# aiforvision/OCTA-autosegmentation

Measured on AMD Instinct MI355X. Metric: synthetic OCTA samples/sec (graph + 304x304 image + 1216x1216 label triples), higher is better.
Workload: dtype f64

## Files before the change

__graft_entry__.py:

```python
import os
import subprocess
import sys

ROOT = os.path.dirname(os.path.abspath(__file__))
if ROOT not in sys.path:
    sys.path.insert(0, ROOT)


def build() -> None:
    from octa_autosegmentation_amd import build as b
    lib = b.build()
    assert os.path.exists(lib)
    from oracle import octa_oracle
    octa_oracle.build()
    nat = os.path.join(ROOT, "tests", "native")
    subprocess.check_call(["g++", "-O2", "-std=c++17", "-ffp-contract=off", "-fPIC", "-shared", "-o",
                           os.path.join(nat, "libcorehost.so"), os.path.join(nat, "raster_core_host.cpp")])
    subprocess.check_call(["g++", "-O2", "-std=c++17", "-mfma", "-ffp-contract=off", "-fPIC", "-shared", "-o",
                           os.path.join(nat, "libsimcorehost.so"), os.path.join(nat, "sim_core_host.cpp")])
    subprocess.check_call(["g++", "-O2", "-std=c++17", "-mfma", "-ffp-contract=off", "-fPIC", "-shared", "-DOCTA_SIM_LARGE=1", "-o",
                           os.path.join(nat, "libsimcorehost_large.so"), os.path.join(nat, "sim_core_host.cpp")])
    import octa_autosegmentation_amd
    from octa_autosegmentation_amd import _native
    assert _native.lib().octa_abi_version() == 2


def smoke() -> None:
    import numpy as np
    import torch
    from octa_autosegmentation_amd.vessel_graph_generation import tree2img
    from oracle import octa_oracle
    assert torch.cuda.is_available(), "smoke() needs a GPU"
    torch.cuda.set_device(0)
    rng = np.random.default_rng(0)
    n = 500
    e = np.zeros((n, 7))
    e[:, 0:3] = rng.uniform(0, 1, (n, 3))
    e[:, 3:6] = e[:, 0:3] + rng.normal(0, 0.03, (n, 3))
    e[:, 6] = rng.uniform(0.001, 0.01, n)
    d = torch.from_numpy(e).cuda()
    img = tree2img.rasterize_edges_device(d, np.array([0, n]), [304, 304])
    lab = tree2img.binarize_label_device(img)
    torch.cuda.synchronize()
    ref = octa_oracle.rasterize(e, [304, 304])
    assert (img[0].cpu().numpy() == ref).all(), "HIP rasteriser differs from the oracle"
    assert (lab[0].cpu().numpy() == octa_oracle.fs_dither(ref)).all(), "HIP dither differs from the oracle"
    import yaml
    from octa_autosegmentation_amd import graph_io
    from octa_autosegmentation_amd.vessel_graph_generation import greenhouse
    from oracle import sim_oracle
    g = np.load(os.path.join(ROOT, "tests", "golden", "sim_golden.npz"))
    cfg = yaml.safe_load(str(g["config_yaml"]))
    cfg["Greenhouse"]["modes"][0]["I"] = 12
    cfg["Greenhouse"]["modes"][1]["I"] = 6
    res = greenhouse.simulate_batch(cfg, [3, 4])
    for k, seed in enumerate((3, 4)):
        e, _ = sim_oracle.simulate(cfg, seed)
        assert graph_io.edges_to_csv_text(res.sample_edges(k)) == sim_oracle.edges_to_csv_text(e), "HIP simulator differs from the oracle"
    import torch.nn.functional as F
    from octa_autosegmentation_amd.models import mfma_conv
    gen = torch.Generator(device="cuda").manual_seed(0)
    x = torch.randn(1, 24, 40, 32, device="cuda", generator=gen).to(torch.bfloat16)
    w = (torch.randn(64, 32, 3, 3, device="cuda", generator=gen) / 17.0).to(torch.bfloat16).float()
    xr, wr = x.float().permute(0, 3, 1, 2).requires_grad_(True), w.clone().requires_grad_(True)
    yr = F.conv2d(xr, wr, padding=1)
    dy = torch.randn(yr.shape, device="cuda", generator=gen).to(torch.bfloat16)
    yr.backward(dy.float())
    xm, wm = x.clone().requires_grad_(True), w.clone().requires_grad_(True)
    ym = mfma_conv.conv3x3(xm, wm, 1)
    ym.backward(dy.permute(0, 2, 3, 1).contiguous())
    tol = lambda a, b: (a.float() - b).abs().max().item() <= 2.0 ** -8 * b.abs().max().item() + 1e-6
    assert tol(ym.detach(), yr.detach().permute(0, 2, 3, 1)), "MFMA convolution differs from torch fp32"
    assert tol(xm.grad, xr.grad.permute(0, 2, 3, 1)), "MFMA data gradient differs from torch fp32"
    assert (wm.grad - wr.grad).abs().max().item() <= 1e-3 * wr.grad.abs().max().item(), "MFMA weight gradient differs from torch fp32"
    print("smoke ok: simulator CSV + raster + dither bit-exact vs oracle, MFMA conv fwd/dgrad/wgrad vs torch fp32, on", torch.cuda.get_device_name(0))


if __name__ == "__main__":
    build()
    if len(sys.argv) > 1 and sys.argv[1] == "smoke":
        smoke()
```

octa_autosegmentation_amd/csrc/sim_core.h:

```cpp
#pragma once
#include <cmath>
#include <cstdint>
#include <cstring>
#include <algorithm>
#include "gpow.h"
#include "glibc_trig.h"

#ifndef OCTA_SIM_LARGE
#define OCTA_SIM_LARGE 0
#endif
#if OCTA_SIM_LARGE
#define OCTA_SIMK octa_simk_large
#else
#define OCTA_SIMK octa_simk
#endif
namespace OCTA_SIMK {

#if OCTA_SIM_LARGE
typedef unsigned int idx_t;
typedef unsigned long long kdw_t;
constexpr int IDX_BITS = 18;
constexpr int GROUP_BITS = 17;
constexpr int NCAP = 1 << 17;
constexpr int OCAP = 1 << 18;
// ... 814 lines not shown
#pragma unroll
        for (int d = 1; d < 64; d <<= 1) {
            int u = __shfl_up(inc, d, 64);
            if (tl >= d) inc += u;
        }
        const int totS = __shfl(inc, 63, 64);
        const int preS = inc - nS;
        const int cut = base + totS;
        {
            int g = (p0 - base) - preS;
            const int lim = p1 < cut ? p1 : cut;
            for (int i = p0; i < lim; i++)
                if (!kd_less_w(a, a.kv[i], pk)) box[g++] = (idx_t)i;
        }
        __builtin_amdgcn_wave_barrier();
        {
            int r = totS - preS - nS;
            const int lo = p0 > cut ? p0 : cut;
            for (int i = p1 - 1; i >= lo; i--)
                if (kd_less_w(a, a.kv[i], pk)) kd_swap(a, i, (int)box[r++]);
        }
        __builtin_amdgcn_wave_barrier();
        if (cut <= nth) first = cut; else last = cut;
    }
    kd_nth_element_team<64, 4>(a, first, nth, last, true, mb, depth);
}
#endif

OCTA_HD inline unsigned f32_bits(float v) { unsigned u; memcpy(&u, &v, 4); return u; }
OCTA_HD inline unsigned f32_sortable(float v) {
    unsigned u;
    memcpy(&u, &v, 4);
    return (u >> 31) ? ~u : (u | 0x80000000u);
}
OCTA_HD inline float f32_unsortable(unsigned e) {
    unsigned u = (e >> 31) ? (e & 0x7fffffffu) : ~e;
    float v;
    memcpy(&v, &u, 4);
    return v;
}
OCTA_HD inline float f32_round_up(double x) {
#if defined(__HIP_DEVICE_COMPILE__)
    return __double2float_ru(x);
#else
    float f = (float)x;
    return (double)f < x ? nextafterf(f, INFINITY) : f;
#endif
}
OCTA_HD inline float f32_round_down(double x) {
#if defined(__HIP_DEVICE_COMPILE__)
    return __double2float_rd(x);
#else
    float f = (float)x;
    return (double)f > x ? nextafterf(f, -INFINITY) : f;
#endif
}
OCTA_HD inline double f32_ulp(float v) {
    const float a = fabsf(v);
    return (double)nextafterf(a, INFINITY) - (double)a;
}
OCTA_HD inline void atomic_max_u32(unsigned *p, unsigned v) {
#if defined(__HIP_DEVICE_COMPILE__)
    atomicMax(p, v);
#else
    if (v > *p) *p = v;
#endif
}
OCTA_HD inline void atomic_min_u32(unsigned *p, unsigned v) {
#if defined(__HIP_DEVICE_COMPILE__)
    atomicMin(p, v);
#else
    if (v < *p) *p = v;
#endif
}

constexpr int KD_TAB_OFF = OCAP * (int)sizeof(kdw_t);
constexpr int KD_BOX_BYTES = KD_RANGES * 24;
static_assert(KD_RANGES >= OCAP / 17 + 1, "ranges per level");
static_assert(KD_MAILBOX_OFF % 16 == 0 && KD_MAILBOX_OFF >= KD_TAB_OFF + KD_RANGES * KD_TAB_BYTES_PER_RANGE, "kd tables overlap the mailbox");
static_assert(KD_MAILBOX_OFF + (KD_BOX_BYTES > KD_MAILBOX_BYTES ? KD_BOX_BYTES : KD_MAILBOX_BYTES) <= SIM_USER_BYTES, "kd table layout (box table and mailbox share their area)");
OCTA_HD inline void kd_build(const Blk &b, const double *pts, int n, idx_t *out_idx, idx_t *out_rank,
                              float *xy, double zlo, double zhi, long *kdprof = nullptr, const unsigned char *need = nullptr,
                              const bool flag_in_sign = false) {
#if defined(__HIP_DEVICE_COMPILE__) && !defined(OCTA_SIM_PROF_ASSIGN) && !defined(OCTA_SIM_PROF_SAMPLE) && !defined(OCTA_SIM_PROF_SET) && !defined(OCTA_SIM_PROF_MAIL) && !defined(OCTA_SIM_PROF_SEQ) && !defined(OCTA_SIM_PROF_SEQ2)
#define KDP(slot) do { if (kdprof && b.tid == 0) { long _t = (long)wall_clock64(); kdprof[slot] += _t - _kt; _kt = _t; } } while (0)
    long _kt = (long)wall_clock64();
#else
#define KDP(slot) do { } while (0)
#endif
    kdw_t *kv = reinterpret_cast<kdw_t *>(b.user_of<1>());
    idx_t *tab = reinterpret_cast<idx_t *>(b.user_of<1>() + KD_TAB_OFF);
    idx_t *rs = tab, *re = tab + KD_RANGES;
    idx_t *rs2 = tab + 2 * KD_RANGES, *re2 = tab + 3 * KD_RANGES;
    signed char *rd = reinterpret_cast<signed char *>(tab + 4 * KD_RANGES);
    unsigned *bbf = reinterpret_cast<unsigned *>(b.user_of<1>() + KD_MAILBOX_OFF);
#if defined(__HIP_DEVICE_COMPILE__) && !OCTA_SIM_LARGE
    if ((size_t)n * (sizeof(kdw_t) + 8) + 8 <= (size_t)KD_TAB_OFF)
        xy = reinterpret_cast<float *>(b.user_of<1>() + (((size_t)n * sizeof(kdw_t) + 7) & ~(size_t)7));
#endif
    for (int i = b.tid; i < n; i += b.nth) {
        kv[i] = (kdw_t)i;
        const float fx = (float)pts[3 * i];
        xy[2 * i] = (flag_in_sign && need[i]) ? -fx : fx; xy[2 * i + 1] = (float)pts[3 * i + 1];
    }
    if (b.tid == 0) { rs[0] = 0; re[0] = (idx_t)n; }
    const float z_up = f32_round_up(zhi), z_dn = f32_round_down(zlo);
    b.sync();
    int nr = (n > 16) ? 1 : 0;
    while (nr > 0) {
        for (int q = b.tid; q < nr; q += b.nth) {
            for (int k = 0; k < 2; k++) { bbf[6 * q + k] = 0u; bbf[6 * q + 3 + k] = ~0u; }
            bbf[6 * q + 2] = f32_sortable(z_up); bbf[6 * q + 5] = f32_sortable(z_dn);
            rd[q] = 0;
        }
        b.sync();
        {
            const int chunk = ((n + b.nth - 1) / b.nth) | 1;
            const int i0 = b.tid * chunk, i1 = (i0 + chunk < n) ? i0 + chunk : n;
            int q = 0;
            if (i0 < i1) {
                int lo_ = 0, hi_ = nr - 1;
                while (lo_ < hi_) { int mid = (lo_ + hi_ + 1) >> 1; if (rs[mid] <= i0) lo_ = mid; else hi_ = mid - 1; }
                q = lo_;
            }
            bool have = false, hit = false;
            float mx[2] = {0, 0}, mn[2] = {0, 0};
            auto flush = [&](int qq) {
                for (int k = 0; k < 2; k++) {
                    atomic_max_u32(&bbf[6 * qq + k], f32_sortable(nextafterf(mx[k], INFINITY)));
                    atomic_min_u32(&bbf[6 * qq + 3 + k], f32_sortable(nextafterf(mn[k], -INFINITY)));
                }
            };
            constexpr int KB = 8;
            int qw = q, cs = 0, ce = 0, ns = 0x7fffffff;
            if (i0 < i1) { cs = rs[qw]; ce = re[qw]; ns = qw + 1 < nr ? (int)rs[qw + 1] : 0x7fffffff; }
            for (int ib = i0; ib < i1; ib += KB) {
                int eq[KB], eid[KB];
                kdw_t ew[KB];
#pragma unroll
                for (int k = 0; k < KB; k++) ew[k] = kv[ib + k < i1 ? ib + k : i1 - 1];
#pragma unroll
                for (int k = 0; k < KB; k++) {
                    const int i = ib + k;
                    eq[k] = -1; eid[k] = 0;
                    if (i < i1) {
                        while (i >= ns) { qw++; cs = ns; ce = re[qw]; ns = qw + 1 < nr ? (int)rs[qw + 1] : 0x7fffffff; }
                        if (i >= cs && i < ce) { eq[k] = qw; eid[k] = (int)(ew[k] & KD_IDX_MASK); }
                    }
                }
                float ex[KB], ey[KB];
                unsigned char nd[KB];
#pragma unroll
                for (int k = 0; k < KB; k++) {
                    const float sx = xy[2 * eid[k]];
                    ex[k] = flag_in_sign ? fabsf(sx) : sx; ey[k] = xy[2 * eid[k] + 1];
                    nd[k] = flag_in_sign ? (unsigned char)(f32_bits(sx) >> 31) : (need ? need[eid[k]] : (unsigned char)1);
                }
#pragma unroll
                for (int k = 0; k < KB; k++) {
                    if (eq[k] < 0) continue;
                    if (eq[k] != q) {
                        if (have) { flush(q); have = false; }
                        if (hit) { rd[q] = 1; hit = false; }
                        q = eq[k];
                    }
                    if (nd[k]) hit = true;
                    if (!have) { mx[0] = mn[0] = ex[k]; mx[1] = mn[1] = ey[k]; }
// ... 110 lines not shown
                }
            }
        }
        b.sync();
        KDP(2);
#if defined(__HIP_DEVICE_COMPILE__)
        {
            idx_t *mb = reinterpret_cast<idx_t *>(b.user_of<1>() + KD_MAILBOX_OFF);
            const int wv = b.tid >> 6, nw = (b.nth + 63) >> 6;
            for (int q = wv; q < nr; q += nw) {
                int d = rd[q];
                int s = rs[q], e = re[q];
                if (d < 0 || e - s < KD_TEAM_MIN) continue;
                const KdPair kp = {kv, pts, d};
                if (e - s > KD_MASK_MAX) kd_nth_element_wave_long(kp, s, s + (e - s) / 2, e, mb);
                else if (e - s > 4000) kd_nth_element_team<64, 4>(kp, s, s + (e - s) / 2, e, true, mb);
                else kd_nth_element_team<64, 1>(kp, s, s + (e - s) / 2, e, true, mb);
            }
        }
        KDP(3);
        {
            idx_t *mb = reinterpret_cast<idx_t *>(b.user_of<1>() + KD_MAILBOX_OFF);
            const int team = b.tid >> 4, nteam = b.nth >> 4;
            for (int q0 = 0; q0 < nr; q0 += nteam) {
                int q = q0 + team;
                bool live = q < nr;
                int s = 0, e = 0, d = 0;
                if (live) {
                    s = rs[q]; e = re[q]; d = rd[q];
                    live = d >= 0 && e - s < KD_TEAM_MIN;
                }
                const KdPair kp = {kv, pts, d < 0 ? 0 : d};
                kd_nth_element_team<16, 1>(kp, s, s + (e - s) / 2, e, live, mb);
            }
        }
#else
        for (int q = b.tid; q < nr; q += b.nth) {
            int d = rd[q];
            if (d < 0) continue;
            int s = rs[q], e = re[q];
            const KdPair kp = {kv, pts, d};
            kd_nth_element(kp, s, s + (e - s) / 2, e);
        }
#endif
        b.sync();
        KDP(4);
        {
            int base = 0;
            for (int q0 = 0; q0 < nr; q0 += b.nth) {
                const int q = q0 + b.tid;
                int s = 0, e = 0, m = 0, c = 0;
                if (q < nr && rd[q] >= 0) {
                    s = rs[q]; e = re[q]; m = s + (e - s) / 2;
                    c = (m - s > 16 ? 1 : 0) + (e - m > 16 ? 1 : 0);
                }
                int ex;
                const int tot = blk_scan(b, c, &ex);
                int pos = base + ex;
                if (m - s > 16) { if (pos < KD_RANGES) { rs2[pos] = (idx_t)s; re2[pos] = (idx_t)m; } pos++; }
                if (e - m > 16) { if (pos < KD_RANGES) { rs2[pos] = (idx_t)m; re2[pos] = (idx_t)e; } }
                base += tot;
            }
            nr = base < KD_RANGES ? base : KD_RANGES;
        }
        { idx_t *t = rs; rs = rs2; rs2 = t; t = re; re = re2; re2 = t; }
        KDP(5);
    }
    for (int i = b.tid; i < n; i += b.nth) { const idx_t id = (idx_t)(kv[i] & KD_IDX_MASK); out_idx[i] = id; out_rank[id] = (idx_t)i; }
    b.sync();
    KDP(6);
#undef KDP
}


constexpr int GRID_N = NCAP > OCAP ? NCAP : OCAP;
struct Grid {
    int nx, ny;
    double x0, y0, inv, cell;
    const int *cell_end;
    const idx_t *items;
    const double *spts;
    const float *sptf;
    const double *src;
};
OCTA_HD inline int grid_clampi(int v, int hi) { return v < 0 ? 0 : (v > hi ? hi : v); }
OCTA_HD inline int grid_cx(const Grid &G, double x) { return grid_clampi((int)floor((x - G.x0) * G.inv), G.nx - 1); }
OCTA_HD inline int grid_cy(const Grid &G, double y) { return grid_clampi((int)floor((y - G.y0) * G.inv), G.ny - 1); }

OCTA_HD inline Grid grid_build_once(const Blk &b, const SimArrays &A, const double *pts, const int *ids, int n, double radius, int div, bool as_float,
                                    const unsigned char *mask) {
    Grid G;
    const double span = 1.2;
    double cell = fmax(radius / div, span / GRID_MAX);
    int nc = (int)ceil(span / cell);
    if (nc < 1) nc = 1;
    if (nc > GRID_MAX) nc = GRID_MAX;
    G.nx = G.ny = nc; G.x0 = G.y0 = -0.1; G.inv = 1.0 / cell; G.cell = cell;
    const int ncell = nc * nc;
    int *hist = reinterpret_cast<int *>(b.user_of<2>());
    idx_t *items = reinterpret_cast<idx_t *>(b.user_of<2>() + (size_t)(GRID_MAX * GRID_MAX + 1) * 4);
    static_assert((size_t)(GRID_MAX * GRID_MAX + 1) * 4 + (size_t)GRID_N * sizeof(idx_t) <= (size_t)SIM_USER_BYTES, "grid table layout");
    G.cell_end = hist; G.items = items; G.spts = A.grid_pts; G.sptf = reinterpret_cast<const float *>(A.grid_pts); G.src = pts;
    if (n > GRID_N) n = GRID_N;
    b.sync();
    for (int c = b.tid; c <= ncell; c += b.nth) hist[c] = 0;
    b.sync();
    constexpr int GB = 4;
    for (int i0 = b.tid; i0 < n; i0 += GB * b.nth) {
        double px[GB], py[GB];
        bool live[GB];
#pragma unroll
        for (int k = 0; k < GB; k++) {
            const int i = i0 + k * b.nth;
            const int ic = i < n ? i : n - 1;
            const double *p = pts + 3 * (ids ? ids[ic] : ic);
            px[k] = p[0]; py[k] = p[1];
            live[k] = i < n && (!mask || mask[ic]);
        }
#pragma unroll
        for (int k = 0; k < GB; k++)
            if (live[k]) atomic_add_int(&hist[grid_cy(G, py[k]) * nc + grid_cx(G, px[k])], 1);
    }
    b.sync();
    {
        const int total = ncell + 1;
        const int chunk = ((total + b.nth - 1) / b.nth) | 1;
        const int c0 = b.tid * chunk, c1 = (c0 + chunk < total) ? c0 + chunk : total;
        int local = 0;
        for (int c = c0; c < c1; c++) local += hist[c];
        int ex;
        blk_scan(b, local, &ex);
        int run = ex;
        for (int c = c0; c < c1; c++) { int v = hist[c]; hist[c] = run; run += v; }
    }
    b.sync();
    for (int i0 = b.tid; i0 < n; i0 += GB * b.nth) {
        V3 p[GB];
        int id[GB];
        bool live[GB];
#pragma unroll
        for (int k = 0; k < GB; k++) {
            const int i = i0 + k * b.nth;
            const int ic = i < n ? i : n - 1;
            id[k] = ids ? ids[ic] : ic;
            p[k] = ld3(pts + 3 * id[k]);
            live[k] = i < n && (!mask || mask[ic]);
        }
#pragma unroll
        for (int k = 0; k < GB; k++)
            if (live[k]) {
                int pos = atomic_add_int(&hist[grid_cy(G, p[k].y) * nc + grid_cx(G, p[k].x)], 1);
                items[pos] = (idx_t)id[k];
                if (as_float) { float *f = reinterpret_cast<float *>(A.grid_pts) + 3 * pos; f[0] = (float)p[k].x; f[1] = (float)p[k].y; f[2] = (float)p[k].z; }
                else st3(A.grid_pts + 3 * pos, p[k]);
            }
    }
    b.sync();
    return G;
}
OCTA_HD inline Grid grid_build(const Blk &b, const SimArrays &A, const double *pts, const int *ids, int n, double radius, int div = 1,
                               bool as_float = false, const unsigned char *mask = nullptr) {
#if OCTA_SIM_DUP & 2
    grid_build_once(b, A, pts, ids, n, radius, div, as_float, mask);
#endif
    return grid_build_once(b, A, pts, ids, n, radius, div, as_float, mask);
}
constexpr int GRID_VB = 4;
constexpr double GRID_F_TAU = 1e-6;
struct Pt3f { float x, y, z; };
OCTA_HD inline float sqdist_f(Pt3f a, float cx, float cy, float cz) { const float dx = a.x - cx, dy = a.y - cy, dz = a.z - cz; return fmaf(dz, dz, fmaf(dy, dy, dx * dx)); }
template <bool FLT> struct GridPt;
template <> struct GridPt<false> { typedef V3 T; static OCTA_HD inline V3 load(const Grid &G, int k) { return ld3(G.spts + 3 * k); } static OCTA_HD inline V3 zero() { return v3(0, 0, 0); } };
template <> struct GridPt<true> {
    typedef Pt3f T;
    static OCTA_HD inline Pt3f load(const Grid &G, int k) { const float *f = G.sptf + 3 * k; Pt3f r = {f[0], f[1], f[2]}; return r; }
    static OCTA_HD inline Pt3f zero() { Pt3f r = {0.f, 0.f, 0.f}; return r; }
};
template <bool FLT, class F>
OCTA_HD inline void grid_visit_impl(const Grid &G, double px, double py, double radius, F &&body) {
    const int cy0 = grid_cy(G, py - radius), cy1 = grid_cy(G, py + radius);
    const int cx0 = grid_cx(G, px - radius), cx1 = grid_cx(G, px + radius);
    for (int cyb = cy0; cyb <= cy1; cyb += 3) {
        int k0[3], k1[3];
#pragma unroll
        for (int r = 0; r < 3; r++) {
            const int row = cyb + r;
            k0[r] = k1[r] = 0;
            if (row <= cy1) {
                const int c0 = row * G.nx + cx0;
                k0[r] = c0 ? G.cell_end[c0 - 1] : 0;
                k1[r] = G.cell_end[row * G.nx + cx1];
            }
        }
        typename GridPt<FLT>::T pt[3][GRID_VB];
        int it[3][GRID_VB];
#pragma unroll
        for (int r = 0; r < 3; r++)
#pragma unroll
            for (int u = 0; u < GRID_VB; u++) {
                const int k = k0[r] + u < k1[r] ? k0[r] + u : k0[r];
                pt[r][u] = k0[r] < k1[r] ? GridPt<FLT>::load(G, k) : GridPt<FLT>::zero();
                it[r][u] = k0[r] < k1[r] ? (int)G.items[k] : 0;
            }
#pragma unroll
        for (int r = 0; r < 3; r++) {
#pragma unroll
            for (int u = 0; u < GRID_VB; u++)
                if (k0[r] + u < k1[r]) body(it[r][u], pt[r][u]);
            for (int kb = k0[r] + GRID_VB; kb < k1[r]; kb += GRID_VB) {
                typename GridPt<FLT>::T q[GRID_VB];
                int iq[GRID_VB];
#pragma unroll
                for (int u = 0; u < GRID_VB; u++) {
                    const int k = kb + u < k1[r] ? kb + u : kb;
                    q[u] = GridPt<FLT>::load(G, k);
                    iq[u] = (int)G.items[k];
                }
#pragma unroll
                for (int u = 0; u < GRID_VB; u++)
                    if (kb + u < k1[r]) body(iq[u], q[u]);
            }
        }
    }
}
template <class F>
OCTA_HD inline void grid_visit(const Grid &G, double px, double py, double radius, F &&body) { grid_visit_impl<false>(G, px, py, radius, body); }
template <class F>
OCTA_HD inline void grid_visit_f(const Grid &G, double px, double py, double radius, F &&body) { grid_visit_impl<true>(G, px, py, radius, body); }

struct DirtyList {
    int *v;
    int n, cap;
    bool overflow;
};
OCTA_HD inline void dirty_insert(DirtyList &D, int g) {
    int i = 0;
    while (i < D.n && D.v[i] < g) i++;
    if (i < D.n && D.v[i] == g) return;
    if (OCTA_UNLIKELY(D.n >= D.cap)) { D.overflow = true; return; }
    for (int k = D.n; k > i; k--) D.v[k] = D.v[k - 1];
    D.v[i] = g;
    D.n++;
}

struct SeqLds {
    double *rad;
    idx_t *par;
    const double *log_tab;
    const uint64_t *exp_tab;
    int *deferred;
    int *changed;
    double *fl_val;
    int *fl_done;
    int *slot_of;
};
#ifndef OCTA_MURRAY_EPT
#define OCTA_MURRAY_EPT 4
#endif
constexpr int MURRAY_EPT = OCTA_MURRAY_EPT;
constexpr int MURRAY_FLUSH_WAVE = MURRAY_EPT * 64;
constexpr int MURRAY_FLUSH_LDS = 3 * MURRAY_FLUSH_WAVE;
constexpr int PAR_BITS = (int)sizeof(idx_t) * 8 - 2;
constexpr unsigned PAR_MASK = (1u << PAR_BITS) - 1u, PAR_DEF = 1u << PAR_BITS, PAR_TAG = 2u << PAR_BITS;
static_assert((unsigned)NCAP <= PAR_MASK, "node ids fit the parent field of a node word");
OCTA_HD inline bool changed_get(const SeqLds &L, int g) { return ((unsigned)L.changed[g >> 5] >> (g & 31)) & 1u; }
OCTA_HD inline void changed_set(const SeqLds &L, int g) { L.changed[g >> 5] |= (int)(1u << (g & 31)); }
OCTA_HD inline bool deferred_get(const SeqLds &L, int id) { return ((unsigned)L.deferred[id >> 5] >> (id & 31)) & 1u; }
struct WalkRec { int nch, c0, c1, cg; double k; };
OCTA_HD inline WalkRec walk_load(const SimArrays &A, int f, int id, bool want_cg) {
    WalkRec r;
    const int j = id < 0 ? 0 : id;
    r.nch = A.nnch_of(f)[j]; r.c0 = A.nch0_of(f)[j]; r.c1 = A.nch1_of(f)[j];
    r.cg = want_cg ? A.child_group[j] : 0;
    r.k = A.nkap_of(f)[j];
    return r;
}
OCTA_HD inline int walk_parent(const SeqLds &L, int id) {
    if (id < 0) return -1;
    const unsigned p = (unsigned)L.par[id] & PAR_MASK;
    return p == PAR_MASK ? -1 : (int)p;
}

#if defined(__HIP_DEVICE_COMPILE__)
__device__ inline double readlane_f64(double v, int j ) {
    int lo = __builtin_amdgcn_readlane(__double2loint(v), j), hi = __builtin_amdgcn_readlane(__double2hiint(v), j);
    return __hiloint2double(hi, lo);
}
__device__ inline bool murray_pending_above(const SimArrays &A, int start, int cur_g, int pass_tag, const SeqLds &L) {
    const int lane = (int)(threadIdx.x & 63);
    int cur = start;
    while (true) {
        int nn = 0, mine = -1;
        bool ended = false;
        for (; nn < 64; nn++) {
            const unsigned w = (unsigned)L.par[cur], p = w & PAR_MASK;
            if (p == PAR_MASK || (w & PAR_DEF)) { ended = true; break; }
            if (lane == nn) mine = cur;
            cur = (int)p;
        }
        const int cg = lane < nn ? A.child_group[mine] : 0;
        if (__ballot(lane < nn && (cg >> (GROUP_BITS + 1)) == pass_tag && (cg & ((1 << GROUP_BITS) - 1)) > cur_g)) return true;
        if (ended) return false;
    }
}
#ifdef OCTA_WALK_POW_LDS
#define OCTA_WALK_POW(x, y) octa_gpow::gpow_t((x), (y), L.log_tab, L.exp_tab)
#else
#define OCTA_WALK_POW(x, y) octa_gpow::gpow_u((x), (y))
#endif
__device__ inline long murray_to_root(const SimArrays &A, int f, int id, int cur_g, int pass_tag, DirtyList *D, const SeqLds &L, int &n_def
#ifdef OCTA_SIM_PROF_SEQ2
// ... 1397 lines not shown
#endif
        }
    }
    b.sync();
}

OCTA_HD inline void murray_flush_pending(const Blk &b, const SimArrays &A) {
#if defined(__HIP_DEVICE_COMPILE__)
    b.sync();
    double *fl_val = reinterpret_cast<double *>(b.user_of<8>());
    int *fl_done = reinterpret_cast<int *>(fl_val + MURRAY_FLUSH_LDS);
    for (int f = 0; f < 2; f++) {
        const int n = OCTA_UNI(A.sc->fl_pending[f]);
        if (n <= 0) continue;
        for (int i = b.tid; i < MURRAY_FLUSH_LDS / 32; i += b.nth) fl_done[i] = 0;
        b.sync();
        const int wv = b.tid >> 6;
        if (wv < 3 && wv * 64 < n) {
            const int rounds = murray_flush_rounds_wave(A.nrad_of(f), octa_gpow::LOG_TAB, octa_gpow::EXP_TAB, fl_val, fl_done, A.fl_rec + (size_t)f * MURRAY_FLUSH_LDS, n,
                                                        wv, 3, true);
            if (b.tid == 0) { A.sc->fl_pending[f] = 0; A.sc->flush_rounds += rounds; }
        }
        b.sync();
    }
#else
    (void)b; (void)A;
#endif
}

constexpr int COMPACT_TILE = 3072;
OCTA_HD inline int compact_points(const Blk &b, double *pts, int n, const unsigned char *removed, double *stage) {
    (void)stage;
    if (b.nth == 1) {
        int w = 0;
        for (int i = 0; i < n; i++)
            if (!removed[i]) { if (w != i) { pts[3 * w] = pts[3 * i]; pts[3 * w + 1] = pts[3 * i + 1]; pts[3 * w + 2] = pts[3 * i + 2]; } w++; }
        return w;
    }
    double *tile = reinterpret_cast<double *>(b.user_of<16>());
    static_assert((size_t)COMPACT_TILE * 24 <= (size_t)SIM_USER_BYTES, "compaction tile");
#if defined(__HIP_DEVICE_COMPILE__)
    const int lane = b.tid & 63, wv = b.tid >> 6, nw = (b.nth + 63) >> 6;
    int base = 0;
    for (int t0 = 0; t0 < n; t0 += COMPACT_TILE) {
        const int tn = n - t0 < COMPACT_TILE ? n - t0 : COMPACT_TILE;
        const int seg = ((tn + nw * 64 - 1) / (nw * 64)) * 64;
        const int s0 = t0 + (wv * seg < tn ? wv * seg : tn), s1 = s0 + seg < t0 + tn ? s0 + seg : t0 + tn;
        int c = 0;
        for (int i0 = s0; i0 < s1; i0 += 64) c += (int)__popcll(__ballot(i0 + lane < s1 && !removed[i0 + lane]));
        int ex;
        const int kept = blk_scan(b, lane == 0 ? c : 0, &ex);
        if (base != t0 || kept != tn) {
            int at = __builtin_amdgcn_readfirstlane(ex);
            for (int i0 = s0; i0 < s1; i0 += 64) {
                const bool keep = i0 + lane < s1 && !removed[i0 + lane];
                const unsigned long long m = __ballot(keep);
                if (keep) {
                    const int w = at + (int)__popcll(m & ((1ull << lane) - 1ull));
                    const V3 v = ld3(pts + 3 * (size_t)(i0 + lane));
                    tile[3 * w] = v.x; tile[3 * w + 1] = v.y; tile[3 * w + 2] = v.z;
                }
                at += (int)__popcll(m);
            }
            b.sync();
            for (int j = b.tid; j < kept * 3; j += b.nth) pts[(size_t)3 * base + j] = tile[j];
            b.sync();
        }
        base += kept;
    }
    return base;
#else
    (void)tile;
    return n;
#endif
}

#if defined(__HIP_DEVICE_COMPILE__)
#define OCTA_SUBPROF(sc, slot, t0) do { if (b.tid == 0) { long _t1 = (long)wall_clock64(); (sc)->prof[slot] += _t1 - (t0); (t0) = _t1; } } while (0)
#define OCTA_SUBPROF_T0() ((long)wall_clock64())
#else
#define OCTA_SUBPROF(sc, slot, t0) do { (void)(t0); } while (0)
#define OCTA_SUBPROF_T0() 0L
#endif

OCTA_HD inline void phase_satisfy_art(const Blk &b, const SimArrays &A, const SimConst &C, const IterParams &P) {
    const double zext = C.sz;
    SampleScalars *sc = A.sc;
    const int nb = sc->new_begin[0], ne = sc->new_end[0];
    const int n_new = ne - nb, n_oxy = sc->n_oxy;
    if (n_new <= 0 || n_oxy <= 0) return;
    const double ek = P.eps_k, ek2 = ek * ek;
    long t0 = OCTA_SUBPROF_T0();
    for (int i = b.tid; i < n_oxy; i += b.nth) A.removed[i] = 0;
    int *ctl = b.coll() + 100;
    if (b.tid == 0) { ctl[0] = 0; ctl[1] = 0; }
    b.sync();
    {
        int *new_ids = A.tmp_int;
        for (int j = b.tid; j < n_new; j += b.nth) new_ids[j] = nb + j;
        b.sync();
        Grid G = grid_build(b, A, A.npos[0], new_ids, n_new, ek);
        for (int o = b.tid; o < n_oxy; o += b.nth) {
            const V3 p = ld3(A.oxy + 3 * o);
            grid_visit(G, p.x, p.y, ek, [&](int j, const V3 &q) {
                if (sqdist(p, q) <= ek2) {
                    int slot = atomic_add_int(&ctl[0], 1);
                    if (slot < PCAP) A.pairs[slot] = ((unsigned)(j - nb) << IDX_BITS) | (unsigned)o;
                    A.removed[o] = 1;
                }
            });
        }
        b.sync();
    }
    OCTA_SUBPROF(sc, 12, t0);
    int n_pairs = ctl[0];
    if (n_pairs > PCAP) { if (b.tid == 0) atomic_or_int(&sc->err, ERR_PAIR_CAP); n_pairs = PCAP; }
    if (n_new > (1 << (32 - IDX_BITS))) { if (b.tid == 0) atomic_or_int(&sc->err, ERR_PAIR_CAP); }
    b.sync();
    if (n_pairs == 0) return;
    {
        const int n_ven = sc->n_nodes[1];
        int *rem = A.tmp_int;
        int n_rem = 0;
        {
            const int chunk = (n_oxy + b.nth - 1) / b.nth;
            const int i0 = b.tid * chunk < n_oxy ? b.tid * chunk : n_oxy, i1 = (i0 + chunk < n_oxy) ? i0 + chunk : n_oxy;
            int local = 0;
            for (int o = i0; o < i1; o++) local += A.removed[o] ? 1 : 0;
            int ex;
            n_rem = blk_scan(b, local, &ex);
            int run = ex;
            for (int o = i0; o < i1; o++) if (A.removed[o]) rem[run++] = o;
        }
        b.sync();
        for (int k = b.tid; k < n_rem; k += b.nth) {
            const int o = rem[k];
            A.ven_near[o] = 0;
            A.hashes[o] = py_hash_tuple3(ld3(A.oxy + 3 * o));
        }
        Grid G = grid_build(b, A, A.oxy, rem, n_rem, ek);
        constexpr int VB = 4;
        for (int j0 = b.tid; j0 < n_ven; j0 += VB * b.nth) {
            V3 qv[VB];
#pragma unroll
            for (int u = 0; u < VB; u++) { const int j = j0 + u * b.nth; qv[u] = ld3(A.npos[1] + 3 * (j < n_ven ? j : n_ven - 1)); }
#pragma unroll
            for (int u = 0; u < VB; u++) {
                if (j0 + u * b.nth >= n_ven) break;
                const V3 q = qv[u];
                grid_visit(G, q.x, q.y, ek, [&](int o, const V3 &p) {
                    if (sqrt(sqdist(q, p)) <= ek) A.ven_near[o] = 1;
                });
            }
        }
        b.sync();
    }
    OCTA_SUBPROF(sc, 12, t0);
    bool set_in_lds = false, ranked = false;
#ifdef OCTA_SIM_DEBUG_SAT
    int dbg_n_ins = -1, dbg_mask = -1, dbg_base = -1;
    const int dbg_n_co2_in = sc->n_co2;
#endif
    for (int pass = 0; pass < 2; pass++) {
        ranked = pass > 0;
        if (ranked) {
            kd_build(b, A.oxy, n_oxy, A.kd_idx, A.kd_rank, reinterpret_cast<float *>(A.tmp_dbl), 0.0, zext, sc->kdprof, A.removed, true);
#if OCTA_SIM_DUP & 1
            kd_build(b, A.oxy, n_oxy, A.kd_idx, A.kd_rank, reinterpret_cast<float *>(A.tmp_dbl), 0.0, zext, nullptr, A.removed, true);
#endif
            for (int i = b.tid; i < n_pairs; i += b.nth) {
                unsigned pr = A.pairs[i];
                A.pairs[i] = (pr & ~IDX_MASK) | (unsigned)A.kd_rank[pr & IDX_MASK];
            }
            b.sync();
            OCTA_SUBPROF(sc, 11, t0);
        }
        unsigned *keys = reinterpret_cast<unsigned *>(b.user_of<32>());
        int n_pow2 = 1;
        while (n_pow2 < n_pairs) n_pow2 <<= 1;
        for (int i = b.tid; i < n_pow2; i += b.nth) keys[i] = i < n_pairs ? A.pairs[i] : 0xffffffffu;
        b.sync();
        if (n_pairs > 0) blk_sort_u32(b, keys, n_pow2);
        for (int i = b.tid; i < n_pairs; i += b.nth) A.pairs[i] = keys[i];
        b.sync();
        OCTA_SUBPROF(sc, 13, t0);
#if defined(__HIP_DEVICE_COMPILE__)
#if defined(OCTA_SIM_PROF_SET)
        long _pt = (long)wall_clock64();
#define PSP(slot) do { if (b.tid == 0) { long _t = (long)wall_clock64(); sc->kdprof[slot] += _t - _pt; _pt = _t; } } while (0)
#else
#define PSP(slot) do { } while (0)
#endif
        constexpr int EMPTY = 0x7fffffff;
        auto replay = [&](int *own, int *in_key, unsigned long long *in_hash, int *dk, unsigned long long *dh, int *ord0, int *ord1,
                          const int s_max) __attribute__((always_inline)) -> int {
            int n_ins = 0;
            for (int p0 = 0; p0 < n_pairs; p0 += b.nth) {
                const int i = p0 + b.tid;
                int o = -1, take = 0;
                unsigned long long hsh = 0;
                if (i < n_pairs) {
                    o = ranked ? (int)A.kd_idx[keys[i] & IDX_MASK] : (int)(keys[i] & IDX_MASK);
                    take = A.ven_near[o] ? 0 : 1;
                    hsh = A.hashes[o];
                }
                int ex;
                const int tot = blk_scan(b, take, &ex);
                if (take) { in_key[n_ins + ex] = (int)((keys[i] & ~IDX_MASK) | (unsigned)o); in_hash[n_ins + ex] = hsh; }
                n_ins += tot;
            }
            b.sync();
            PSP(0);
            for (int i = b.tid; i < n_ins; i += b.nth) own[(unsigned)in_key[i] & IDX_MASK] = EMPTY;
            b.sync();
            for (int i = b.tid; i < n_ins; i += b.nth) atomic_min_int(&own[(unsigned)in_key[i] & IDX_MASK], i);
            b.sync();
            int D = 0;
            for (int p0 = 0; p0 < n_ins; p0 += b.nth) {
                const int i = p0 + b.tid;
                const bool first = i < n_ins && own[(unsigned)in_key[i] & IDX_MASK] == i;
                int ex;
                const int tot = blk_scan(b, first ? 1 : 0, &ex);
                if (first) { dk[D + ex] = in_key[i]; dh[D + ex] = in_hash[i]; }
                D += tot;
            }
            b.sync();
            PSP(1);
            int S = 8, n_prev = 0;
            int *ord = ord0, *ord_next = ord1;
            while (true) {
                const int thr = (3 * (S - 1) + 4) / 5;
                const int upto = D < thr ? D : thr;
                const unsigned long long mask = (unsigned long long)(S - 1);
                for (int p = n_prev + b.tid; p < upto; p += b.nth) ord[p] = p;
                for (int e = b.tid; e < S; e += b.nth) own[e] = EMPTY;
                b.sync();
                for (int p = b.tid; p < upto; p += b.nth) {
                    int cur = p;
// ... 156 lines not shown
            }
            if (!ranked && !pyset_order_free(cw, cw + OCAP, A.hashes, D, cw + 4 * OCAP, cw + 2 * OCAP, cw + 3 * OCAP, SETCAP / 2)) ctl[1] = 1;
            if (ranked || !ctl[1]) {
                int n_co2 = sc->n_co2;
                for (int e = 0; e <= S.mask; e++)
                    if (S.key[e] >= 0) {
                        if (n_co2 >= CCAP) { sc->err |= ERR_CO2_CAP; break; }
                        int o = S.key[e];
                        A.co2[3 * n_co2] = A.oxy[3 * o]; A.co2[3 * n_co2 + 1] = A.oxy[3 * o + 1]; A.co2[3 * n_co2 + 2] = A.oxy[3 * o + 2];
                        n_co2++;
                    }
                sc->n_co2 = n_co2;
            }
        }
        b.sync();
        OCTA_SUBPROF(sc, 14, t0);
        if (!ranked && ctl[1]) continue;
        if (b.tid == 0) sc->kd_path[ranked ? 1 : 0]++;
        break;
    }
#if defined(OCTA_SIM_DEBUG_SAT) && !defined(OCTA_SIM_ITER_PROF)
    {
        int ex, loc;
        loc = 0; for (int o = b.tid; o < n_oxy; o += b.nth) loc += A.removed[o] ? 1 : 0;
        const int c_rem = blk_scan(b, loc, &ex);
        loc = 0; for (int o = b.tid; o < n_oxy; o += b.nth) loc += (A.removed[o] && A.ven_near[o]) ? 1 : 0;
        const int c_ven = blk_scan(b, loc, &ex);
        unsigned char *mark = reinterpret_cast<unsigned char *>(A.tmp_dbl);
        for (int o = b.tid; o < 2 * n_oxy; o += b.nth) mark[o] = 0;
        b.sync();
        for (int i = b.tid; i < n_pairs; i += b.nth) {
            const int o = ranked ? (int)A.kd_idx[A.pairs[i] & IDX_MASK] : (int)(A.pairs[i] & IDX_MASK);
            mark[o] = 1;
            if (!A.ven_near[o]) mark[n_oxy + o] = 1;
        }
        b.sync();
        loc = 0; for (int o = b.tid; o < n_oxy; o += b.nth) loc += mark[o];
        const int c_pair_all = blk_scan(b, loc, &ex);
        loc = 0; for (int o = b.tid; o < n_oxy; o += b.nth) loc += mark[n_oxy + o];
        const int c_pair_take = blk_scan(b, loc, &ex);
        loc = 0; for (int o = b.tid; o < n_oxy; o += b.nth) loc += (mark[o] != (A.removed[o] ? 1 : 0)) ? 1 : 0;
        const int c_pair_vs_removed = blk_scan(b, loc, &ex);
        int c_slots = -1, c_in_distinct = -1, c_slot_bad = -1;
        if (set_in_lds) {
            const int *t_key = reinterpret_cast<const int *>(b.user());
            const int *in_key = t_key + (OCAP > LSET_CAP / 2 ? OCAP : LSET_CAP / 2);
            loc = 0; for (int e = b.tid; e <= dbg_mask; e += b.nth) loc += t_key[e] >= 0 ? 1 : 0;
            c_slots = blk_scan(b, loc, &ex);
            loc = 0; for (int e = b.tid; e <= dbg_mask; e += b.nth) { const int k = t_key[e]; if (k >= 0 && (k >= n_oxy || !A.removed[k] || A.ven_near[k])) loc++; }
            c_slot_bad = blk_scan(b, loc, &ex);
            for (int o = b.tid; o < n_oxy; o += b.nth) mark[o] = 0;
            b.sync();
            for (int i = b.tid; i < dbg_n_ins; i += b.nth) { const int k = (int)((unsigned)in_key[i] & IDX_MASK); if (k < n_oxy) mark[k] = 1; }
            b.sync();
            loc = 0; for (int o = b.tid; o < n_oxy; o += b.nth) loc += mark[o];
            c_in_distinct = blk_scan(b, loc, &ex);
        }
        b.sync();
        if (b.tid == 0 && A.dbg) {
            int *row = A.dbg + 16 * A.dbg_it;
            row[0] = n_new; row[1] = n_oxy; row[2] = n_pairs; row[3] = c_rem; row[4] = c_ven; row[5] = c_pair_all; row[6] = c_pair_take;
            row[7] = c_pair_vs_removed; row[8] = dbg_n_ins; row[9] = dbg_mask; row[10] = dbg_base; row[11] = c_slots; row[12] = c_in_distinct;
            row[13] = c_slot_bad; row[14] = dbg_n_co2_in; row[15] = sc->n_co2;
        }
        b.sync();
    }
#endif
    int keep = compact_points(b, A.oxy, n_oxy, A.removed, A.tmp_dbl);
    if (b.tid == 0) sc->n_oxy = keep;
    b.sync();
    OCTA_SUBPROF(sc, 15, t0);
}

OCTA_HD inline void phase_satisfy_ven(const Blk &b, const SimArrays &A, const IterParams &P) {
    SampleScalars *sc = A.sc;
    const int nb = sc->new_begin[1], ne = sc->new_end[1];
    const int n_new = ne - nb, n_co2 = sc->n_co2;
    if (n_new <= 0 || n_co2 <= 0) return;
    const double ek2 = P.eps_k * P.eps_k;
    const double ek = P.eps_k;
    {
        int *new_ids = A.tmp_int;
        for (int j = b.tid; j < n_new; j += b.nth) new_ids[j] = nb + j;
        b.sync();
        Grid G = grid_build(b, A, A.npos[1], new_ids, n_new, ek);
        for (int o = b.tid; o < n_co2; o += b.nth) {
            const V3 p = ld3(A.co2 + 3 * o);
            bool hit = false;
            grid_visit(G, p.x, p.y, ek, [&](int, const V3 &q) {
                if (!hit && sqdist(p, q) <= ek2) hit = true;
            });
            A.removed[o] = hit ? 1 : 0;
        }
        b.sync();
    }
    int keep = compact_points(b, A.co2, n_co2, A.removed, A.tmp_dbl);
    if (b.tid == 0) sc->n_co2 = keep;
    b.sync();
}

}
```

Before: 1395.

## Use sparse-occupancy grid build with reach bitmap to skip far queries

Adds a sparse grid builder that tracks cell occupancy bits so the prefix scan and empty-cell fill touch only occupied cells, and marks a reach bitmap of cells within the search radius of any inserted point. Queries in the three satisfy phases first test this bitmap and skip grid traversal for points that cannot hit anything. The aim is to cut the cost of building grids over small new-node sets and of visiting neighbours for mostly-distant query points. In exchange it adds atomics over the reach footprint at build time and more shared-memory layout constraints, with a fallback when n exceeds the sparse capacity.

```diff
diff --git a/__graft_entry__.py b/__graft_entry__.py
--- a/__graft_entry__.py
+++ b/__graft_entry__.py
@@ -20,6 +20,10 @@
                            os.path.join(nat, "libsimcorehost.so"), os.path.join(nat, "sim_core_host.cpp")])
     subprocess.check_call(["g++", "-O2", "-std=c++17", "-mfma", "-ffp-contract=off", "-fPIC", "-shared", "-DOCTA_SIM_LARGE=1", "-o",
                            os.path.join(nat, "libsimcorehost_large.so"), os.path.join(nat, "sim_core_host.cpp")])
+    subprocess.check_call(["g++", "-O2", "-std=c++17", "-mfma", "-ffp-contract=off", "-fPIC", "-shared", "-o",
+                           os.path.join(nat, "libsparsegridhost.so"), os.path.join(nat, "sparse_grid_host.cpp")])
+    subprocess.check_call(["g++", "-O2", "-std=c++17", "-mfma", "-ffp-contract=off", "-fPIC", "-shared", "-DOCTA_SIM_LARGE=1", "-o",
+                           os.path.join(nat, "libsparsegridhost_large.so"), os.path.join(nat, "sparse_grid_host.cpp")])
     import octa_autosegmentation_amd
     from octa_autosegmentation_amd import _native
     assert _native.lib().octa_abi_version() == 2
diff --git a/octa_autosegmentation_amd/csrc/sim_core.h b/octa_autosegmentation_amd/csrc/sim_core.h
--- a/octa_autosegmentation_amd/csrc/sim_core.h
+++ b/octa_autosegmentation_amd/csrc/sim_core.h
@@ -920,7 +920,7 @@
 OCTA_HD inline void kd_build(const Blk &b, const double *pts, int n, idx_t *out_idx, idx_t *out_rank,
                               float *xy, double zlo, double zhi, long *kdprof = nullptr, const unsigned char *need = nullptr,
                               const bool flag_in_sign = false) {
-#if defined(__HIP_DEVICE_COMPILE__) && !defined(OCTA_SIM_PROF_ASSIGN) && !defined(OCTA_SIM_PROF_SAMPLE) && !defined(OCTA_SIM_PROF_SET) && !defined(OCTA_SIM_PROF_MAIL) && !defined(OCTA_SIM_PROF_SEQ) && !defined(OCTA_SIM_PROF_SEQ2)
+#if defined(__HIP_DEVICE_COMPILE__) && !defined(OCTA_SIM_PROF_ASSIGN) && !defined(OCTA_SIM_PROF_SAMPLE) && !defined(OCTA_SIM_PROF_SET) && !defined(OCTA_SIM_PROF_MAIL) && !defined(OCTA_SIM_PROF_SEQ) && !defined(OCTA_SIM_PROF_SEQ2) && !defined(OCTA_SIM_PROF_SPARSE)
 #define KDP(slot) do { if (kdprof && b.tid == 0) { long _t = (long)wall_clock64(); kdprof[slot] += _t - _kt; _kt = _t; } } while (0)
     long _kt = (long)wall_clock64();
 #else
@@ -1197,6 +1197,7 @@
     const double *spts;
     const float *sptf;
     const double *src;
+    const unsigned *bits;
 };
 OCTA_HD inline int grid_clampi(int v, int hi) { return v < 0 ? 0 : (v > hi ? hi : v); }
 OCTA_HD inline int grid_cx(const Grid &G, double x) { return grid_clampi((int)floor((x - G.x0) * G.inv), G.nx - 1); }
@@ -1215,7 +1216,7 @@
     int *hist = reinterpret_cast<int *>(b.user_of<2>());
     idx_t *items = reinterpret_cast<idx_t *>(b.user_of<2>() + (size_t)(GRID_MAX * GRID_MAX + 1) * 4);
     static_assert((size_t)(GRID_MAX * GRID_MAX + 1) * 4 + (size_t)GRID_N * sizeof(idx_t) <= (size_t)SIM_USER_BYTES, "grid table layout");
-    G.cell_end = hist; G.items = items; G.spts = A.grid_pts; G.sptf = reinterpret_cast<const float *>(A.grid_pts); G.src = pts;
+    G.cell_end = hist; G.items = items; G.spts = A.grid_pts; G.sptf = reinterpret_cast<const float *>(A.grid_pts); G.src = pts; G.bits = nullptr;
     if (n > GRID_N) n = GRID_N;
     b.sync();
     for (int c = b.tid; c <= ncell; c += b.nth) hist[c] = 0;
@@ -1342,6 +1343,137 @@
 OCTA_HD inline void grid_visit(const Grid &G, double px, double py, double radius, F &&body) { grid_visit_impl<false>(G, px, py, radius, body); }
 template <class F>
 OCTA_HD inline void grid_visit_f(const Grid &G, double px, double py, double radius, F &&body) { grid_visit_impl<true>(G, px, py, radius, body); }
+
+constexpr int GRID_BITS_WORDS = (GRID_MAX * GRID_MAX + 31) / 32;
+constexpr size_t GRID_ITEMS_OFF = (size_t)(GRID_MAX * GRID_MAX + 1) * 4;
+constexpr size_t GRID_BITS_OFF = ((size_t)SIM_USER_BYTES - (size_t)GRID_BITS_WORDS * 4) & ~(size_t)15;
+constexpr int GRID_SPARSE_N = (GRID_BITS_OFF - GRID_ITEMS_OFF) / sizeof(idx_t) < (size_t)GRID_N ? (int)((GRID_BITS_OFF - GRID_ITEMS_OFF) / sizeof(idx_t)) : GRID_N;
+constexpr double GRID_REACH_MARGIN = 1e-9;
+static_assert(GRID_ITEMS_OFF % 4 == 0 && GRID_ITEMS_OFF + (size_t)2 * GRID_BITS_WORDS * 4 <= GRID_BITS_OFF && GRID_SPARSE_N >= 1 &&
+              GRID_BITS_OFF + (size_t)GRID_BITS_WORDS * 4 <= (size_t)SIM_USER_BYTES, "sparse grid table layout (occupancy + word ends over the items, reach bitmap behind them)");
+static_assert((GRID_MAX * GRID_MAX) % 4 == 0, "the offsets of empty cells are filled four at a time");
+OCTA_HD inline int grid_ctz(unsigned m) { return __builtin_ctz(m); }
+struct alignas(16) GridInt4 { int a, b, c, d; };
+OCTA_HD inline void grid_store4(int *p, int v) {
+#if defined(__HIP_DEVICE_COMPILE__)
+    *reinterpret_cast<GridInt4 *>(p) = GridInt4{v, v, v, v};
+#else
+    p[0] = v; p[1] = v; p[2] = v; p[3] = v;
+#endif
+}
+OCTA_HD inline Grid grid_build_sparse(const Blk &b, const SimArrays &A, const double *pts, const int *ids, int n, double radius) {
+    Grid G;
+    const double span = 1.2;
+    double cell = fmax(radius, span / GRID_MAX);
+    int nc = (int)ceil(span / cell);
+    if (nc < 1) nc = 1;
+    if (nc > GRID_MAX) nc = GRID_MAX;
+    G.nx = G.ny = nc; G.x0 = G.y0 = -0.1; G.inv = 1.0 / cell; G.cell = cell;
+    const int ncell = nc * nc, nw = (ncell + 31) >> 5;
+    int *hist = reinterpret_cast<int *>(b.user_of<2>());
+    idx_t *items = reinterpret_cast<idx_t *>(b.user_of<2>() + GRID_ITEMS_OFF);
+    unsigned *occ = reinterpret_cast<unsigned *>(b.user_of<2>() + GRID_ITEMS_OFF);
+    int *wend = reinterpret_cast<int *>(occ + GRID_BITS_WORDS);
+    unsigned *bits = reinterpret_cast<unsigned *>(b.user_of<2>() + GRID_BITS_OFF);
+    const bool use_bits = n <= GRID_SPARSE_N;
+    G.cell_end = hist; G.items = items; G.spts = A.grid_pts; G.sptf = reinterpret_cast<const float *>(A.grid_pts); G.src = pts;
+    G.bits = use_bits ? bits : nullptr;
+    if (n > GRID_N) n = GRID_N;
+    constexpr int GB = 4;
+    auto cell_of = [&](int i) { const double *p = pts + 3 * ids[i]; return grid_cy(G, p[1]) * nc + grid_cx(G, p[0]); };
+    b.sync();
+    for (int w = b.tid; w < nw; w += b.nth) { occ[w] = 0; if (use_bits) bits[w] = 0; }
+    for (int c = 4 * b.tid; c < ncell; c += 4 * b.nth) grid_store4(hist + c, 0);
+    b.sync();
+    for (int i = b.tid; i < n; i += b.nth) {
+        const int c = cell_of(i);
+        atomic_add_int(&hist[c], 1);
+        atomic_or_int(reinterpret_cast<int *>(&occ[c >> 5]), (int)(1u << (c & 31)));
+    }
+    b.sync();
+    {
+        const int wchunk = (nw + b.nth - 1) / b.nth;
+        const int w0 = b.tid * wchunk < nw ? b.tid * wchunk : nw, w1 = w0 + wchunk < nw ? w0 + wchunk : nw;
+        int local = 0;
+        for (int w = w0; w < w1; w++)
+            for (unsigned m = occ[w]; m; m &= m - 1) local += hist[w * 32 + grid_ctz(m)];
+        int ex;
+        blk_scan(b, local, &ex);
+        int run = ex;
+        for (int w = w0; w < w1; w++) {
+            for (unsigned m = occ[w]; m; m &= m - 1) { const int c = w * 32 + grid_ctz(m); const int v = hist[c]; hist[c] = run; run += v; }
+            wend[w] = run;
+        }
+    }
+    b.sync();
+    for (int c = 4 * b.tid; c < ncell; c += 4 * b.nth) {
+        const int w = c >> 5;
+        const unsigned hi = occ[w] >> (c & 31);
+        if (!OCTA_UNLIKELY(hi & 15u)) {
+            const int e = hi ? hist[c + grid_ctz(hi)] : wend[w];
+            grid_store4(hist + c, e);
+        } else {
+            int e = (hi >> 4) ? hist[c + 4 + grid_ctz(hi >> 4)] : wend[w];
+            for (int k = 3; k >= 0; k--) { if ((hi >> k) & 1u) e = hist[c + k]; else hist[c + k] = e; }
+        }
+    }
+    b.sync();
+    const double reach = radius + GRID_REACH_MARGIN;
+    for (int i0 = b.tid; i0 < n; i0 += GB * b.nth) {
+        V3 p[GB];
+        int id[GB];
+#pragma unroll
+        for (int k = 0; k < GB; k++) {
+            const int i = i0 + k * b.nth;
+            id[k] = ids[i < n ? i : n - 1];
+            p[k] = ld3(pts + 3 * id[k]);
+        }
+#pragma unroll
+        for (int k = 0; k < GB; k++)
+            if (i0 + k * b.nth < n) {
+                const int c = grid_cy(G, p[k].y) * nc + grid_cx(G, p[k].x);
+                const int pos = atomic_add_int(&hist[c], 1);
+                items[pos] = (idx_t)id[k];
+                st3(A.grid_pts + 3 * pos, p[k]);
+                if (use_bits) {
+                    const int bx0 = grid_cx(G, p[k].x - reach), bx1 = grid_cx(G, p[k].x + reach);
+                    const int by0 = grid_cy(G, p[k].y - reach), by1 = grid_cy(G, p[k].y + reach);
+                    for (int row = by0; row <= by1; row++)
+                        for (int cc = row * nc + bx0; cc <= row * nc + bx1; cc++)
+                            atomic_or_int(reinterpret_cast<int *>(&bits[cc >> 5]), (int)(1u << (cc & 31)));
+                }
+            }
+    }
+    b.sync();
+    return G;
+}
+OCTA_HD inline bool grid_reach(const Grid &G, double px, double py) {
+    if (!G.bits) return true;
+    const int c = grid_cy(G, py) * G.nx + grid_cx(G, px);
+    return (G.bits[c >> 5] >> (c & 31)) & 1u;
+}
+template <class F>
+OCTA_HD inline void grid_stream_sparse(const Blk &b, const Grid &G, const double *q, int nq, double radius, F &&body) {
+    constexpr int VB = 4;
+    for (int j0 = b.tid; j0 < nq; j0 += VB * b.nth) {
+        double qx[VB], qy[VB];
+#pragma unroll
+        for (int u = 0; u < VB; u++) {
+            const int j = j0 + u * b.nth;
+            const double *p = q + 3 * (size_t)(j < nq ? j : nq - 1);
+            qx[u] = p[0]; qy[u] = p[1];
+        }
+        unsigned m = 0;
+#pragma unroll
+        for (int u = 0; u < VB; u++)
+            if (j0 + u * b.nth < nq && grid_reach(G, qx[u], qy[u])) m |= 1u << u;
+        for (; OCTA_UNLIKELY(m != 0); m &= m - 1) {
+            const int j = j0 + grid_ctz(m) * b.nth;
+            const V3 p = ld3(q + 3 * (size_t)j);
+            grid_visit(G, p.x, p.y, radius, [&](int item, const V3 &g) { body(j, p, item, g); });
+        }
+    }
+}
 
 struct DirtyList {
     int *v;
@@ -2905,6 +3037,11 @@
 #define OCTA_SUBPROF(sc, slot, t0) do { (void)(t0); } while (0)
 #define OCTA_SUBPROF_T0() 0L
 #endif
+#if defined(OCTA_SIM_PROF_SPARSE) && defined(__HIP_DEVICE_COMPILE__)
+#define OCTA_SPARSEPROF(sc, slot, t) do { if (b.tid == 0) { long _t1 = (long)wall_clock64(); (sc)->kdprof[slot] += _t1 - (t); (t) = _t1; } } while (0)
+#else
+#define OCTA_SPARSEPROF(sc, slot, t) do { (void)(t); } while (0)
+#endif
 
 OCTA_HD inline void phase_satisfy_art(const Blk &b, const SimArrays &A, const SimConst &C, const IterParams &P) {
     const double zext = C.sz;
@@ -2922,18 +3059,18 @@
         int *new_ids = A.tmp_int;
         for (int j = b.tid; j < n_new; j += b.nth) new_ids[j] = nb + j;
         b.sync();
-        Grid G = grid_build(b, A, A.npos[0], new_ids, n_new, ek);
-        for (int o = b.tid; o < n_oxy; o += b.nth) {
-            const V3 p = ld3(A.oxy + 3 * o);
-            grid_visit(G, p.x, p.y, ek, [&](int j, const V3 &q) {
-                if (sqdist(p, q) <= ek2) {
-                    int slot = atomic_add_int(&ctl[0], 1);
-                    if (slot < PCAP) A.pairs[slot] = ((unsigned)(j - nb) << IDX_BITS) | (unsigned)o;
-                    A.removed[o] = 1;
-                }
-            });
-        }
+        long ts = OCTA_SUBPROF_T0();
+        Grid G = grid_build_sparse(b, A, A.npos[0], new_ids, n_new, ek);
+        OCTA_SPARSEPROF(sc, 0, ts);
+        grid_stream_sparse(b, G, A.oxy, n_oxy, ek, [&](int o, const V3 &p, int j, const V3 &q) {
+            if (sqdist(p, q) <= ek2) {
+                int slot = atomic_add_int(&ctl[0], 1);
+                if (slot < PCAP) A.pairs[slot] = ((unsigned)(j - nb) << IDX_BITS) | (unsigned)o;
+                A.removed[o] = 1;
+            }
+        });
         b.sync();
+        OCTA_SPARSEPROF(sc, 1, ts);
     }
     OCTA_SUBPROF(sc, 12, t0);
     int n_pairs = ctl[0];
@@ -2945,6 +3082,7 @@
         const int n_ven = sc->n_nodes[1];
         int *rem = A.tmp_int;
         int n_rem = 0;
+        long ts = OCTA_SUBPROF_T0();
         {
             const int chunk = (n_oxy + b.nth - 1) / b.nth;
             const int i0 = b.tid * chunk < n_oxy ? b.tid * chunk : n_oxy, i1 = (i0 + chunk < n_oxy) ? i0 + chunk : n_oxy;
@@ -2961,22 +3099,14 @@
             A.ven_near[o] = 0;
             A.hashes[o] = py_hash_tuple3(ld3(A.oxy + 3 * o));
         }
-        Grid G = grid_build(b, A, A.oxy, rem, n_rem, ek);
-        constexpr int VB = 4;
-        for (int j0 = b.tid; j0 < n_ven; j0 += VB * b.nth) {
-            V3 qv[VB];
-#pragma unroll
-            for (int u = 0; u < VB; u++) { const int j = j0 + u * b.nth; qv[u] = ld3(A.npos[1] + 3 * (j < n_ven ? j : n_ven - 1)); }
-#pragma unroll
-            for (int u = 0; u < VB; u++) {
-                if (j0 + u * b.nth >= n_ven) break;
-                const V3 q = qv[u];
-                grid_visit(G, q.x, q.y, ek, [&](int o, const V3 &p) {
-                    if (sqrt(sqdist(q, p)) <= ek) A.ven_near[o] = 1;
-                });
-            }
-        }
+        OCTA_SPARSEPROF(sc, 2, ts);
+        Grid G = grid_build_sparse(b, A, A.oxy, rem, n_rem, ek);
+        OCTA_SPARSEPROF(sc, 3, ts);
+        grid_stream_sparse(b, G, A.npos[1], n_ven, ek, [&](int, const V3 &q, int o, const V3 &p) {
+            if (sqrt(sqdist(q, p)) <= ek) A.ven_near[o] = 1;
+        });
         b.sync();
+        OCTA_SPARSEPROF(sc, 4, ts);
     }
     OCTA_SUBPROF(sc, 12, t0);
     bool set_in_lds = false, ranked = false;
@@ -3299,17 +3429,16 @@
     {
         int *new_ids = A.tmp_int;
         for (int j = b.tid; j < n_new; j += b.nth) new_ids[j] = nb + j;
+        for (int o = b.tid; o < n_co2; o += b.nth) A.removed[o] = 0;
         b.sync();
-        Grid G = grid_build(b, A, A.npos[1], new_ids, n_new, ek);
-        for (int o = b.tid; o < n_co2; o += b.nth) {
-            const V3 p = ld3(A.co2 + 3 * o);
-            bool hit = false;
-            grid_visit(G, p.x, p.y, ek, [&](int, const V3 &q) {
-                if (!hit && sqdist(p, q) <= ek2) hit = true;
-            });
-            A.removed[o] = hit ? 1 : 0;
-        }
+        long ts = OCTA_SUBPROF_T0();
+        Grid G = grid_build_sparse(b, A, A.npos[1], new_ids, n_new, ek);
+        OCTA_SPARSEPROF(sc, 5, ts);
+        grid_stream_sparse(b, G, A.co2, n_co2, ek, [&](int o, const V3 &p, int, const V3 &q) {
+            if (sqdist(p, q) <= ek2) A.removed[o] = 1;
+        });
         b.sync();
+        OCTA_SPARSEPROF(sc, 6, ts);
     }
     int keep = compact_points(b, A.co2, n_co2, A.removed, A.tmp_dbl);
     if (b.tid == 0) sc->n_co2 = keep;
```

Result: no change. 1410, median of 6 (+1.1%).
